# Drexubery/ViewCrafter

Measured on NVIDIA H100. Metric: DDIM denoise-steps/sec @ 576x1024x25f, higher is better.
Workload: dtype f16 (fp32 accumulate; fp32 norms/softmax/update)

## Files before the change

### viewcrafter_b200/csrc/attention.cu

```cuda
#include <cstdlib>

#include "common.cuh"
#include "kernels.h"
#include "wgmma.cuh"

namespace vc {

struct AttnParams {
  CUtensorMap tmap_q, tmap_k, tmap_v;
  __half* out;
  int ldo;
  int Nq, Nk;
  int kv_shared;
  float scale_log2;
  int accumulate;
};

static constexpr int ATT_BM = 128, ATT_D = 64;
static constexpr int ATT_THREADS = 288;
static constexpr int ATT_Q_BYTES = ATT_BM * ATT_D * 2;

template <int BNK>
struct AttnCfg {
  static constexpr int KV_BYTES = BNK * ATT_D * 2;
  static constexpr int SMEM = ATT_Q_BYTES + 4 * KV_BYTES + 1024 + 256;
  static constexpr int MIN_CTAS = BNK == 64 ? 2 : 1;
};

__device__ __forceinline__ float ex2f(float x) {
  float y;
  asm("ex2.approx.ftz.f32 %0, %1;" : "=f"(y) : "f"(x));
  return y;
}

template <int BNK>
__global__ void __launch_bounds__(ATT_THREADS, AttnCfg<BNK>::MIN_CTAS) flash_attn_d64_kernel(const __grid_constant__ AttnParams p) {
  using Cfg = AttnCfg<BNK>;
  extern __shared__ uint8_t smem_raw[];
  uint8_t* smem = reinterpret_cast<uint8_t*>((reinterpret_cast<uintptr_t>(smem_raw) + 1023) & ~uintptr_t(1023));
  uint8_t* sQ = smem;
  uint8_t* sKV = smem + ATT_Q_BYTES;
  uint64_t* bars = reinterpret_cast<uint64_t*>(smem + ATT_Q_BYTES + 4 * Cfg::KV_BYTES);
  uint64_t* q_full = bars + 0;
  uint64_t* kv_full = bars + 1;
  uint64_t* kv_empty = bars + 3;

  const int warp = threadIdx.x >> 5, lane = threadIdx.x & 31;
  const int q0 = blockIdx.x * ATT_BM, head = blockIdx.y, b = blockIdx.z;
  const int bk = p.kv_shared ? 0 : b;
  const int ntiles = (p.Nk + BNK - 1) / BNK;

  if (threadIdx.x == 0) {
    tma_prefetch_desc(&p.tmap_q);
    tma_prefetch_desc(&p.tmap_k);
    tma_prefetch_desc(&p.tmap_v);
    mbar_init(q_full, 1);
    mbar_init(&kv_full[0], 1); mbar_init(&kv_full[1], 1);
    mbar_init(&kv_empty[0], 8); mbar_init(&kv_empty[1], 8);
    fence_barrier_init();
  }
  __syncthreads();

  if (warp == 8) {
    if (elect_one()) {
      mbar_expect_tx(q_full, ATT_Q_BYTES);
      tma_load_4d(sQ, &p.tmap_q, q_full, 0, head, q0, b);
    }
    __syncwarp();
    for (int j = 0; j < ntiles; ++j) {
      const int s = j & 1;
      uint8_t* sk = sKV + s * 2 * Cfg::KV_BYTES;
      if (j >= 2) mbar_wait(&kv_empty[s], ((j >> 1) - 1) & 1);
      if (elect_one()) {
        mbar_expect_tx(&kv_full[s], 2 * Cfg::KV_BYTES);
        tma_load_4d(sk, &p.tmap_k, &kv_full[s], 0, head, j * BNK, bk);
        tma_load_4d(sk + Cfg::KV_BYTES, &p.tmap_v, &kv_full[s], 0, head, j * BNK, bk);
      }
      __syncwarp();
    }
    return;
  }

  const int cw = warp >> 2, wl = warp & 3;
  const uint32_t aQ = smem_u32(sQ) + cw * (64 * ATT_D * 2);
  const float sl2 = p.scale_log2;
  float o[32];
#pragma unroll
  for (int i = 0; i < 32; ++i) o[i] = 0.f;
  float m[2] = {-INFINITY, -INFINITY}, l[2] = {0.f, 0.f};
  mbar_wait(q_full, 0);
  for (int j = 0; j < ntiles; ++j) {
    const int s = j & 1;
    const uint32_t aK = smem_u32(sKV + s * 2 * Cfg::KV_BYTES);
    const uint32_t aV = aK + Cfg::KV_BYTES;
    mbar_wait(&kv_full[s], (j >> 1) & 1);
    float sc[BNK / 2];
    wgmma_fence();
#pragma unroll
    for (int k = 0; k < ATT_D / 16; ++k) Wgmma<BNK>::ss(sc, wgmma_desc_sw128(aQ + 32 * k), wgmma_desc_sw128(aK + 32 * k), k > 0 ? 1 : 0);
    wgmma_commit();
    wgmma_wait<0>();
    wgmma_fence_regs(sc);

    const int valid = p.Nk - j * BNK;
    if (valid < BNK) {
#pragma unroll
      for (int i = 0; i < BNK / 2; ++i) {
        const int col = 8 * (i >> 2) + 2 * (lane & 3) + (i & 1);
        if (col >= valid) sc[i] = -INFINITY;
      }
    }
    float mx[2] = {-INFINITY, -INFINITY};
#pragma unroll
    for (int i = 0; i < BNK / 2; ++i) mx[(i >> 1) & 1] = fmaxf(mx[(i >> 1) & 1], sc[i]);
    float alpha[2], negm[2];
#pragma unroll
    for (int h = 0; h < 2; ++h) {
      mx[h] = fmaxf(mx[h], __shfl_xor_sync(0xffffffffu, mx[h], 1));
      mx[h] = fmaxf(mx[h], __shfl_xor_sync(0xffffffffu, mx[h], 2));
      const float mn = fmaxf(m[h], mx[h] * sl2);
      alpha[h] = ex2f(m[h] - mn);
      m[h] = mn;
      negm[h] = -mn;
      l[h] *= alpha[h];
    }
#pragma unroll
    for (int i = 0; i < 32; ++i) o[i] *= alpha[(i >> 1) & 1];
    uint32_t pa[BNK / 16][4];
#pragma unroll
    for (int kk = 0; kk < BNK / 16; ++kk) {
#pragma unroll
      for (int r = 0; r < 4; ++r) {
        const int i = (2 * kk + (r >> 1)) * 4 + 2 * (r & 1);
        const int h = r & 1;
        const float e0 = ex2f(fmaf(sc[i], sl2, negm[h])), e1 = ex2f(fmaf(sc[i + 1], sl2, negm[h]));
        l[h] += e0 + e1;
        pa[kk][r] = pack_half2(e0, e1);
      }
    }
    wgmma_fence();
#pragma unroll
    for (int kk = 0; kk < BNK / 16; ++kk) Wgmma<64, 1>::rs(o, pa[kk], wgmma_desc_sw128(aV + kk * 16 * 128), 1);
    wgmma_commit();
    wgmma_wait<0>();
    wgmma_fence_regs(o);
    __syncwarp();
    if (lane == 0) mbar_arrive(&kv_empty[s]);
  }

  float inv[2];
#pragma unroll
  for (int h = 0; h < 2; ++h) {
    float t = l[h];
    t += __shfl_xor_sync(0xffffffffu, t, 1);
    t += __shfl_xor_sync(0xffffffffu, t, 2);
    inv[h] = 1.f / t;
  }
#pragma unroll
  for (int h = 0; h < 2; ++h) {
    const int row = q0 + cw * 64 + 16 * wl + (lane >> 2) + 8 * h;
    if (row >= p.Nq) continue;
    __half* op = p.out + ((long long)b * p.Nq + row) * p.ldo + head * ATT_D + 2 * (lane & 3);
#pragma unroll
    for (int jj = 0; jj < 8; ++jj) {
      float v0 = o[jj * 4 + 2 * h] * inv[h], v1 = o[jj * 4 + 2 * h + 1] * inv[h];
      __half2* dst = reinterpret_cast<__half2*>(op + 8 * jj);
      if (p.accumulate) {
        const float2 t = __half22float2(*dst);
        v0 += t.x; v1 += t.y;
      }
      *dst = __floats2half2_rn(v0, v1);
    }
  }
}

static int bn64_mode() {
  static int mode = -2;
  if (mode == -2) { const char* e = getenv("VC_ATTN_BN64"); mode = !e ? -1 : (e[0] == '1' ? 1 : 0); }
  return mode;
}

template <int BNK>
static int launch_attn(const AttnDesc& d, cudaStream_t stream) {
  using Cfg = AttnCfg<BNK>;
  AttnParams p;
  memset(&p, 0, sizeof(p));
  {
    uint64_t dims[4] = {64, (uint64_t)d.heads, (uint64_t)d.Nq, (uint64_t)d.B};
    uint64_t str[3] = {128, (uint64_t)d.ldq * 2, (uint64_t)d.ldq * 2 * d.Nq};
    uint32_t box[4] = {64, 1, ATT_BM, 1};
    int rc = encode_tmap_f16(&p.tmap_q, d.q, 4, dims, str, box);
    if (rc) return rc;
  }
  const int shared = d.kv_batch_stride == 0;
  {
    uint64_t dims[4] = {64, (uint64_t)d.heads, (uint64_t)d.Nk, (uint64_t)(shared ? 1 : d.B)};
    uint64_t strk[3] = {128, (uint64_t)d.ldk * 2, (uint64_t)(shared ? (long long)d.ldk * d.Nk : d.kv_batch_stride) * 2};
    uint64_t strv[3] = {128, (uint64_t)d.ldv * 2, (uint64_t)(shared ? (long long)d.ldv * d.Nk : d.kv_batch_stride) * 2};
    uint32_t box[4] = {64, 1, (uint32_t)BNK, 1};
    int rc = encode_tmap_f16(&p.tmap_k, d.k, 4, dims, strk, box);
    if (rc) return rc;
    rc = encode_tmap_f16(&p.tmap_v, d.v, 4, dims, strv, box);
    if (rc) return rc;
  }
  p.out = d.out; p.ldo = d.ldo; p.Nq = d.Nq; p.Nk = d.Nk; p.kv_shared = shared;
  p.scale_log2 = d.scale * 1.4426950408889634f;
  p.accumulate = d.accumulate;
  static DeviceOnce configured;
  if (device_once_needed(configured)) {
    VC_CHECK_CUDA(cudaFuncSetAttribute(flash_attn_d64_kernel<BNK>, cudaFuncAttributeMaxDynamicSharedMemorySize, Cfg::SMEM));
    device_once_mark(configured);
  }
  dim3 grid((d.Nq + ATT_BM - 1) / ATT_BM, d.heads, d.B);
  flash_attn_d64_kernel<BNK><<<grid, ATT_THREADS, Cfg::SMEM, stream>>>(p);
  VC_CHECK_CUDA(cudaGetLastError());
  return VC_OK;
}

int flash_attn_d64(const AttnDesc& d, cudaStream_t stream) {
  VC_REQUIRE(d.q && d.k && d.v && d.out, "flash_attn: null pointer");
  VC_REQUIRE(d.Nq > 0 && d.Nk > 0 && d.B > 0 && d.heads > 0, "flash_attn: empty problem");
  VC_REQUIRE(d.ldq % 8 == 0 && d.ldk % 8 == 0 && d.ldv % 8 == 0 && d.ldo % 8 == 0, "flash_attn: pitches must be multiples of 8");
  VC_REQUIRE(d.kv_batch_stride % 8 == 0, "flash_attn: kv batch stride must be a multiple of 8");
  const int mode = bn64_mode();
  if (mode == 1 || (mode < 0 && d.Nk <= 1024)) return launch_attn<64>(d, stream);
  return launch_attn<128>(d, stream);
}

}
```

Baseline: 2.436.

## Add ping-pong warpgroup schedule with 3-stage KV ring for BN128 attention

Adds a separate BN=128 flash-attention kernel with one producer warpgroup and two consumer warpgroups. The consumers alternate tensor-core issue through named barriers, and each one overlaps the next tile's QK^T with the current PV product and softmax. It also adds a third KV stage and a setmaxnreg split (producer 24, MMA warps 240). The aim is to hide softmax/exp latency behind WGMMA and keep TMA further ahead, at the cost of more shared memory and a more complex barrier protocol. The BN=64 path is unchanged.

```diff
diff --git a/viewcrafter_b200/csrc/attention.cu b/viewcrafter_b200/csrc/attention.cu
--- a/viewcrafter_b200/csrc/attention.cu
+++ b/viewcrafter_b200/csrc/attention.cu
@@ -17,15 +17,19 @@
 };
 
 static constexpr int ATT_BM = 128, ATT_D = 64;
-static constexpr int ATT_THREADS = 288;
 static constexpr int ATT_Q_BYTES = ATT_BM * ATT_D * 2;
 
 template <int BNK>
 struct AttnCfg {
+  static constexpr bool PINGPONG = BNK == 128;
+  static constexpr int THREADS = PINGPONG ? 384 : 288;
+  static constexpr int STAGES = PINGPONG ? 3 : 2;
   static constexpr int KV_BYTES = BNK * ATT_D * 2;
-  static constexpr int SMEM = ATT_Q_BYTES + 4 * KV_BYTES + 1024 + 256;
-  static constexpr int MIN_CTAS = BNK == 64 ? 2 : 1;
+  static constexpr int SMEM = ATT_Q_BYTES + STAGES * 2 * KV_BYTES + 1024 + 256;
+  static constexpr int MIN_CTAS = PINGPONG ? 1 : 2;
 };
+static constexpr int ATT_LAUNCH_REGS = 168, ATT_PRODUCER_REGS = 24, ATT_MMA_REGS = 240;
+static_assert(128 * ATT_PRODUCER_REGS + 256 * ATT_MMA_REGS <= ATT_LAUNCH_REGS * AttnCfg<128>::THREADS, "register split exceeds the CTA's allocation");
 
 __device__ __forceinline__ float ex2f(float x) {
   float y;
@@ -34,8 +38,103 @@
 }
 
 template <int BNK>
-__global__ void __launch_bounds__(ATT_THREADS, AttnCfg<BNK>::MIN_CTAS) flash_attn_d64_kernel(const __grid_constant__ AttnParams p) {
+__device__ __forceinline__ void issue_qk(float (&sc)[BNK / 2], uint32_t aQ, uint32_t aK) {
+#pragma unroll
+  for (int k = 0; k < ATT_D / 16; ++k) Wgmma<BNK>::ss(sc, wgmma_desc_sw128(aQ + 32 * k), wgmma_desc_sw128(aK + 32 * k), k > 0 ? 1 : 0);
+}
+
+template <int BNK>
+__device__ __forceinline__ void issue_pv(float (&o)[32], const uint32_t (&pa)[BNK / 16][4], uint32_t aV) {
+#pragma unroll
+  for (int kk = 0; kk < BNK / 16; ++kk) Wgmma<64, 1>::rs(o, pa[kk], wgmma_desc_sw128(aV + kk * 16 * 128), 1);
+}
+
+template <int BNK>
+__device__ __forceinline__ void softmax_tile(float (&sc)[BNK / 2], float (&m)[2], float (&l)[2], float (&alpha)[2], int valid,
+                                             float sl2, int lane) {
+  if (valid < BNK) {
+#pragma unroll
+    for (int i = 0; i < BNK / 2; ++i) {
+      const int col = 8 * (i >> 2) + 2 * (lane & 3) + (i & 1);
+      if (col >= valid) sc[i] = -INFINITY;
+    }
+  }
+  float mx[2] = {-INFINITY, -INFINITY};
+#pragma unroll
+  for (int i = 0; i < BNK / 2; ++i) mx[(i >> 1) & 1] = fmaxf(mx[(i >> 1) & 1], sc[i]);
+  float negm[2];
+#pragma unroll
+  for (int h = 0; h < 2; ++h) {
+    mx[h] = fmaxf(mx[h], __shfl_xor_sync(0xffffffffu, mx[h], 1));
+    mx[h] = fmaxf(mx[h], __shfl_xor_sync(0xffffffffu, mx[h], 2));
+    const float mn = fmaxf(m[h], mx[h] * sl2);
+    alpha[h] = ex2f(m[h] - mn);
+    m[h] = mn;
+    negm[h] = -mn;
+    l[h] *= alpha[h];
+  }
+#pragma unroll
+  for (int kk = 0; kk < BNK / 16; ++kk) {
+#pragma unroll
+    for (int r = 0; r < 4; ++r) {
+      const int i = (2 * kk + (r >> 1)) * 4 + 2 * (r & 1);
+      const int h = r & 1;
+      const float e0 = ex2f(fmaf(sc[i], sl2, negm[h])), e1 = ex2f(fmaf(sc[i + 1], sl2, negm[h]));
+      l[h] += e0 + e1;
+      sc[i] = e0;
+      sc[i + 1] = e1;
+    }
+  }
+}
+
+template <int BNK>
+__device__ __forceinline__ void pack_p(uint32_t (&pa)[BNK / 16][4], const float (&e)[BNK / 2]) {
+#pragma unroll
+  for (int kk = 0; kk < BNK / 16; ++kk) {
+#pragma unroll
+    for (int r = 0; r < 4; ++r) {
+      const int i = (2 * kk + (r >> 1)) * 4 + 2 * (r & 1);
+      pa[kk][r] = pack_half2(e[i], e[i + 1]);
+    }
+  }
+}
+
+__device__ __forceinline__ void rescale_o(float (&o)[32], const float (&alpha)[2]) {
+#pragma unroll
+  for (int i = 0; i < 32; ++i) o[i] *= alpha[(i >> 1) & 1];
+}
+
+__device__ __forceinline__ void store_o(const AttnParams& p, const float (&o)[32], const float (&l)[2], int row0, int b, int head, int lane) {
+  float inv[2];
+#pragma unroll
+  for (int h = 0; h < 2; ++h) {
+    float t = l[h];
+    t += __shfl_xor_sync(0xffffffffu, t, 1);
+    t += __shfl_xor_sync(0xffffffffu, t, 2);
+    inv[h] = 1.f / t;
+  }
+#pragma unroll
+  for (int h = 0; h < 2; ++h) {
+    const int row = row0 + (lane >> 2) + 8 * h;
+    if (row >= p.Nq) continue;
+    __half* op = p.out + ((long long)b * p.Nq + row) * p.ldo + head * ATT_D + 2 * (lane & 3);
+#pragma unroll
+    for (int jj = 0; jj < 8; ++jj) {
+      float v0 = o[jj * 4 + 2 * h] * inv[h], v1 = o[jj * 4 + 2 * h + 1] * inv[h];
+      __half2* dst = reinterpret_cast<__half2*>(op + 8 * jj);
+      if (p.accumulate) {
+        const float2 t = __half22float2(*dst);
+        v0 += t.x; v1 += t.y;
+      }
+      *dst = __floats2half2_rn(v0, v1);
+    }
+  }
+}
+
+template <int BNK>
+__global__ void __launch_bounds__(AttnCfg<BNK>::THREADS, AttnCfg<BNK>::MIN_CTAS) flash_attn_d64_kernel(const __grid_constant__ AttnParams p) {
   using Cfg = AttnCfg<BNK>;
+  static_assert(!Cfg::PINGPONG && Cfg::STAGES == 2, "serial schedule: two stages, 288 threads");
   extern __shared__ uint8_t smem_raw[];
   uint8_t* smem = reinterpret_cast<uint8_t*>((reinterpret_cast<uintptr_t>(smem_raw) + 1023) & ~uintptr_t(1023));
   uint8_t* sQ = smem;
@@ -83,7 +182,6 @@
 
   const int cw = warp >> 2, wl = warp & 3;
   const uint32_t aQ = smem_u32(sQ) + cw * (64 * ATT_D * 2);
-  const float sl2 = p.scale_log2;
   float o[32];
 #pragma unroll
   for (int i = 0; i < 32; ++i) o[i] = 0.f;
@@ -96,82 +194,145 @@
     mbar_wait(&kv_full[s], (j >> 1) & 1);
     float sc[BNK / 2];
     wgmma_fence();
-#pragma unroll
-    for (int k = 0; k < ATT_D / 16; ++k) Wgmma<BNK>::ss(sc, wgmma_desc_sw128(aQ + 32 * k), wgmma_desc_sw128(aK + 32 * k), k > 0 ? 1 : 0);
+    issue_qk<BNK>(sc, aQ, aK);
     wgmma_commit();
     wgmma_wait<0>();
     wgmma_fence_regs(sc);
-
-    const int valid = p.Nk - j * BNK;
-    if (valid < BNK) {
-#pragma unroll
-      for (int i = 0; i < BNK / 2; ++i) {
-        const int col = 8 * (i >> 2) + 2 * (lane & 3) + (i & 1);
-        if (col >= valid) sc[i] = -INFINITY;
-      }
-    }
-    float mx[2] = {-INFINITY, -INFINITY};
-#pragma unroll
-    for (int i = 0; i < BNK / 2; ++i) mx[(i >> 1) & 1] = fmaxf(mx[(i >> 1) & 1], sc[i]);
-    float alpha[2], negm[2];
-#pragma unroll
-    for (int h = 0; h < 2; ++h) {
-      mx[h] = fmaxf(mx[h], __shfl_xor_sync(0xffffffffu, mx[h], 1));
-      mx[h] = fmaxf(mx[h], __shfl_xor_sync(0xffffffffu, mx[h], 2));
-      const float mn = fmaxf(m[h], mx[h] * sl2);
-      alpha[h] = ex2f(m[h] - mn);
-      m[h] = mn;
-      negm[h] = -mn;
-      l[h] *= alpha[h];
-    }
-#pragma unroll
-    for (int i = 0; i < 32; ++i) o[i] *= alpha[(i >> 1) & 1];
+    float alpha[2];
+    softmax_tile<BNK>(sc, m, l, alpha, p.Nk - j * BNK, p.scale_log2, lane);
+    rescale_o(o, alpha);
     uint32_t pa[BNK / 16][4];
-#pragma unroll
-    for (int kk = 0; kk < BNK / 16; ++kk) {
-#pragma unroll
-      for (int r = 0; r < 4; ++r) {
-        const int i = (2 * kk + (r >> 1)) * 4 + 2 * (r & 1);
-        const int h = r & 1;
-        const float e0 = ex2f(fmaf(sc[i], sl2, negm[h])), e1 = ex2f(fmaf(sc[i + 1], sl2, negm[h]));
-        l[h] += e0 + e1;
-        pa[kk][r] = pack_half2(e0, e1);
-      }
-    }
+    pack_p<BNK>(pa, sc);
     wgmma_fence();
-#pragma unroll
-    for (int kk = 0; kk < BNK / 16; ++kk) Wgmma<64, 1>::rs(o, pa[kk], wgmma_desc_sw128(aV + kk * 16 * 128), 1);
+    issue_pv<BNK>(o, pa, aV);
     wgmma_commit();
     wgmma_wait<0>();
     wgmma_fence_regs(o);
     __syncwarp();
     if (lane == 0) mbar_arrive(&kv_empty[s]);
   }
-
-  float inv[2];
-#pragma unroll
-  for (int h = 0; h < 2; ++h) {
-    float t = l[h];
-    t += __shfl_xor_sync(0xffffffffu, t, 1);
-    t += __shfl_xor_sync(0xffffffffu, t, 2);
-    inv[h] = 1.f / t;
-  }
-#pragma unroll
-  for (int h = 0; h < 2; ++h) {
-    const int row = q0 + cw * 64 + 16 * wl + (lane >> 2) + 8 * h;
-    if (row >= p.Nq) continue;
-    __half* op = p.out + ((long long)b * p.Nq + row) * p.ldo + head * ATT_D + 2 * (lane & 3);
-#pragma unroll
-    for (int jj = 0; jj < 8; ++jj) {
-      float v0 = o[jj * 4 + 2 * h] * inv[h], v1 = o[jj * 4 + 2 * h + 1] * inv[h];
-      __half2* dst = reinterpret_cast<__half2*>(op + 8 * jj);
-      if (p.accumulate) {
-        const float2 t = __half22float2(*dst);
-        v0 += t.x; v1 += t.y;
+  store_o(p, o, l, q0 + cw * 64 + 16 * wl, b, head, lane);
+}
+
+__global__ void __launch_bounds__(AttnCfg<128>::THREADS, 1) flash_attn_d64_pingpong_kernel(const __grid_constant__ AttnParams p) {
+  constexpr int BNK = 128;
+  using Cfg = AttnCfg<BNK>;
+  constexpr int STAGES = Cfg::STAGES;
+  extern __shared__ uint8_t smem_raw[];
+  uint8_t* smem = reinterpret_cast<uint8_t*>((reinterpret_cast<uintptr_t>(smem_raw) + 1023) & ~uintptr_t(1023));
+  uint8_t* sQ = smem;
+  uint8_t* sKV = smem + ATT_Q_BYTES;
+  uint64_t* bars = reinterpret_cast<uint64_t*>(smem + ATT_Q_BYTES + STAGES * 2 * Cfg::KV_BYTES);
+  uint64_t* q_full = bars + 0;
+  uint64_t* kv_full = bars + 1;
+  uint64_t* kv_empty = bars + 1 + STAGES;
+
+  const int warp = threadIdx.x >> 5, lane = threadIdx.x & 31;
+  const int q0 = blockIdx.x * ATT_BM, head = blockIdx.y, b = blockIdx.z;
+  const int ntiles = (p.Nk + BNK - 1) / BNK;
+
+  if (threadIdx.x == 0) {
+    tma_prefetch_desc(&p.tmap_q);
+    tma_prefetch_desc(&p.tmap_k);
+    tma_prefetch_desc(&p.tmap_v);
+    mbar_init(q_full, 1);
+    for (int s = 0; s < STAGES; ++s) {
+      mbar_init(&kv_full[s], 1);
+      mbar_init(&kv_empty[s], 8);
+    }
+    fence_barrier_init();
+  }
+  __syncthreads();
+
+  if (warp < 4) {
+    setmaxnreg_dec<ATT_PRODUCER_REGS>();
+    if (warp != 0) return;
+    const int bk = p.kv_shared ? 0 : b;
+    if (elect_one()) {
+      mbar_expect_tx(q_full, ATT_Q_BYTES);
+      tma_load_4d(sQ, &p.tmap_q, q_full, 0, head, q0, b);
+    }
+    __syncwarp();
+    int s = 0;
+    uint32_t ph = 0;
+    for (int j = 0; j < ntiles; ++j) {
+      mbar_wait(&kv_empty[s], ph ^ 1);
+      if (elect_one()) {
+        uint8_t* sk = sKV + s * 2 * Cfg::KV_BYTES;
+        mbar_expect_tx(&kv_full[s], 2 * Cfg::KV_BYTES);
+        tma_load_4d(sk, &p.tmap_k, &kv_full[s], 0, head, j * BNK, bk);
+        tma_load_4d(sk + Cfg::KV_BYTES, &p.tmap_v, &kv_full[s], 0, head, j * BNK, bk);
       }
-      *dst = __floats2half2_rn(v0, v1);
-    }
-  }
+      __syncwarp();
+      if (++s == STAGES) { s = 0; ph ^= 1; }
+    }
+    return;
+  }
+
+  setmaxnreg_inc<ATT_MMA_REGS>();
+  const int cw = (warp >> 2) - 1, wl = warp & 3;
+  const uint32_t aQ = smem_u32(sQ) + cw * (64 * ATT_D * 2);
+  const uint32_t ring = smem_u32(sKV);
+  const float sl2 = p.scale_log2;
+  float o[32];
+#pragma unroll
+  for (int i = 0; i < 32; ++i) o[i] = 0.f;
+  float m[2] = {-INFINITY, -INFINITY}, l[2] = {0.f, 0.f};
+  float sc[BNK / 2];
+  uint32_t pa[BNK / 16][4];
+  float alpha[2];
+  mbar_wait(q_full, 0);
+
+  mbar_wait(&kv_full[0], 0);
+  if (cw == 1) named_bar_sync(2, 256);
+  wgmma_fence();
+  issue_qk<BNK>(sc, aQ, ring);
+  wgmma_commit();
+  named_bar_arrive(2 - cw, 256);
+  wgmma_wait<0>();
+  wgmma_fence_regs(sc);
+  softmax_tile<BNK>(sc, m, l, alpha, p.Nk, sl2, lane);
+  pack_p<BNK>(pa, sc);
+
+  if (ntiles > 1) mbar_wait(&kv_full[1], 0);
+  int s = 0;
+  uint32_t ph = 0;
+  for (int j = 0; j + 1 < ntiles; ++j) {
+    const int s1 = s + 1 == STAGES ? 0 : s + 1;
+    const uint32_t ph1 = s1 == 0 ? ph ^ 1 : ph;
+    const int s2 = s1 + 1 == STAGES ? 0 : s1 + 1;
+    const uint32_t ph2 = s2 == 0 ? ph1 ^ 1 : ph1;
+    const uint32_t aK1 = ring + s1 * 2 * Cfg::KV_BYTES;
+    const uint32_t aV = ring + s * 2 * Cfg::KV_BYTES + Cfg::KV_BYTES;
+    named_bar_sync(1 + cw, 256);
+    wgmma_fence();
+    issue_qk<BNK>(sc, aQ, aK1);
+    wgmma_commit();
+    issue_pv<BNK>(o, pa, aV);
+    wgmma_commit();
+    named_bar_arrive(2 - cw, 256);
+    wgmma_wait<1>();
+    wgmma_fence_regs(sc);
+    softmax_tile<BNK>(sc, m, l, alpha, p.Nk - (j + 1) * BNK, sl2, lane);
+    if (j + 2 < ntiles) mbar_wait(&kv_full[s2], ph2);
+    wgmma_wait<0>();
+    wgmma_fence_regs(o);
+    rescale_o(o, alpha);
+    __syncwarp();
+    if (lane == 0) mbar_arrive(&kv_empty[s]);
+    pack_p<BNK>(pa, sc);
+    s = s1;
+    ph = ph1;
+  }
+
+  named_bar_sync(1 + cw, 256);
+  wgmma_fence();
+  issue_pv<BNK>(o, pa, ring + s * 2 * Cfg::KV_BYTES + Cfg::KV_BYTES);
+  wgmma_commit();
+  if (cw == 0) named_bar_arrive(2, 256);
+  wgmma_wait<0>();
+  wgmma_fence_regs(o);
+  store_o(p, o, l, q0 + cw * 64 + 16 * wl, b, head, lane);
 }
 
 static int bn64_mode() {
@@ -206,13 +367,16 @@
   p.out = d.out; p.ldo = d.ldo; p.Nq = d.Nq; p.Nk = d.Nk; p.kv_shared = shared;
   p.scale_log2 = d.scale * 1.4426950408889634f;
   p.accumulate = d.accumulate;
+  void (*kernel)(AttnParams);
+  if constexpr (Cfg::PINGPONG) kernel = flash_attn_d64_pingpong_kernel;
+  else kernel = flash_attn_d64_kernel<BNK>;
   static DeviceOnce configured;
   if (device_once_needed(configured)) {
-    VC_CHECK_CUDA(cudaFuncSetAttribute(flash_attn_d64_kernel<BNK>, cudaFuncAttributeMaxDynamicSharedMemorySize, Cfg::SMEM));
+    VC_CHECK_CUDA(cudaFuncSetAttribute(kernel, cudaFuncAttributeMaxDynamicSharedMemorySize, Cfg::SMEM));
     device_once_mark(configured);
   }
   dim3 grid((d.Nq + ATT_BM - 1) / ATT_BM, d.heads, d.B);
-  flash_attn_d64_kernel<BNK><<<grid, ATT_THREADS, Cfg::SMEM, stream>>>(p);
+  kernel<<<grid, Cfg::THREADS, Cfg::SMEM, stream>>>(p);
   VC_CHECK_CUDA(cudaGetLastError());
   return VC_OK;
 }
```

New measurement: 2.473, median of 6. 1.5% higher.
